# 0xMiden/miden-vm

Measured on NVIDIA H100. Metric: trace cells/sec proved, higher is better.
Workload: dtype u64

## Files before the change

miden-vm_b200/csrc/kernels.cu:

```cuda
#include "kernels.cuh"
#include "poseidon2.cuh"
#include "poseidon2_fast2.cuh"
#include "ntt2.cuh"
#include "blake3.cuh"
#include "keccak.cuh"
#include "rescue.cuh"
#include <algorithm>
#include <cstdio>

namespace mk {

static unsigned long long g_launches = 0;
unsigned long long launch_count() { return g_launches; }
void count_launch() { ++g_launches; }
void reset_launch_count() { g_launches = 0; }
#define COUNT_LAUNCH() (++g_launches)

void upload_constants() {
    cudaMemcpyToSymbol(p2::D_RC_EXT_INITIAL, p2::P2_RC_EXT_INITIAL, sizeof(u64) * 48);
    cudaMemcpyToSymbol(p2::D_RC_INTERNAL, p2::P2_RC_INTERNAL, sizeof(u64) * 22);
    cudaMemcpyToSymbol(p2::D_RC_EXT_TERMINAL, p2::P2_RC_EXT_TERMINAL, sizeof(u64) * 48);
    cudaMemcpyToSymbol(rsc::D_ARK1, rsc::RESCUE_ARK1, sizeof(u64) * 84);
    cudaMemcpyToSymbol(rsc::D_ARK2, rsc::RESCUE_ARK2, sizeof(u64) * 84);
}
// ... 51 lines not shown
        }
    }
}
void launch_push(const u64* src, const PeerPtrs& dst, u32 rank, u32 world, size_t n, cudaStream_t st) {
    if (!n || world <= 1) return;
    PushArgs a; a.src = src; a.dst = dst; a.rank = rank; a.world = world; a.n = n;
    unsigned blocks = (unsigned)std::min<size_t>((n / 2 + 255) / 256 + 1, 132 * 8);
    k_push<<<blocks, 256, 0, st>>>(a);
    COUNT_LAUNCH();
}

struct TransposeDst { PeerPtrs dst; PeerPtrs bad; u32 world; };
__global__ void k_transpose(const u64* __restrict__ src, TransposeDst d, u32 n_rows, u32 width, size_t col_stride, u32 row0) {
    __shared__ u64 tile[32][33];
    u32 r0 = blockIdx.x * 32, c0 = blockIdx.y * 32;
    bool any_bad = false;
    for (u32 i = threadIdx.y; i < 32; i += 8) {
        u32 r = r0 + i, c = c0 + threadIdx.x;
        if (r < n_rows && c < width) {
            u64 v = src[(size_t)r * width + c];
            any_bad |= (v >= gl::P);
            tile[i][threadIdx.x] = v;
        }
    }
    if (any_bad) for (u32 g = 0; g < d.world; g++) if (d.bad.p[g]) atomicOr(reinterpret_cast<u32*>(d.bad.p[g]), 1u);
    __syncthreads();
    for (u32 i = threadIdx.y; i < 32; i += 8) {
        u32 c = c0 + i, r = r0 + threadIdx.x;
        if (r < n_rows && c < width) {
            u64 v = tile[threadIdx.x][i];
            size_t o = (size_t)c * col_stride + row0 + r;
            for (u32 g = 0; g < d.world; g++) d.dst.p[g][o] = v;
        }
    }
}
void launch_transpose_rm_to_cm(const u64* src, u64* dst, u32 n_rows, u32 width, u32* d_bad_flag, cudaStream_t st) {
    TransposeDst d{}; d.dst.p[0] = dst; d.bad.p[0] = reinterpret_cast<u64*>(d_bad_flag); d.world = 1;
    dim3 grid((n_rows + 31) / 32, (width + 31) / 32), block(32, 8);
    k_transpose<<<grid, block, 0, st>>>(src, d, n_rows, width, (size_t)n_rows, 0u);
    COUNT_LAUNCH();
}
void launch_transpose_slice_push(const u64* src_slice, const PeerPtrs& dst_cm, const PeerPtrs& bad, u32 world, u32 row0, u32 n_rows_slice,
                                 u32 n_rows_total, u32 width, cudaStream_t st) {
    if (!n_rows_slice || !width) return;
    TransposeDst d{}; d.dst = dst_cm; d.bad = bad; d.world = world;
    dim3 grid((n_rows_slice + 31) / 32, (width + 31) / 32), block(32, 8);
    k_transpose<<<grid, block, 0, st>>>(src_slice, d, n_rows_slice, width, (size_t)n_rows_total, row0);
    COUNT_LAUNCH();
}

static constexpr int NTT_THREADS = 256;
static inline unsigned ntt_threads(u32 m, u32 log_cols) {
    u32 g = (m + log_cols >= 3) ? (1u << (m + log_cols - 3)) : 1u;
    if (g < 32) g = 32;
    if (g > 256) g = 256;
    return g;
}

__device__ __forceinline__ u64 w_pow(const u64* __restrict__ hi, const u64* __restrict__ lo, u32 lo_bits, u64 e) {
    return gl::mul(hi[e >> lo_bits], lo[e & ((1ull << lo_bits) - 1)]);
}

#define NTT_BOUNDS __launch_bounds__(NTT_THREADS)
template <int N1C, int N2C>
__global__ void NTT_BOUNDS k_intt_strided(u64* cols, size_t col_stride, NttTables T, u32 log_c) {
    extern __shared__ u64 sm[];
    ntt2::intt_strided_block<N1C, N2C>(blockIdx.x, blockIdx.y, sm, cols, col_stride, T, log_c);
}
template <int N2C>
__global__ void NTT_BOUNDS k_intt_contig(u64* cols, size_t col_stride, NttTables T) {
    extern __shared__ u64 sm[];
    ntt2::intt_contig_block<N2C>(blockIdx.x, blockIdx.y, sm, cols, col_stride, T);
}
template <int N1C, int N2C>
__global__ void NTT_BOUNDS k_fwd_contig(const FwdItem* __restrict__ items, NttTables T, PremulTables Pm) {
    extern __shared__ u64 sm[];
    ntt2::fwd_contig_block<N1C, N2C>(blockIdx.x, blockIdx.y, sm, items, T, Pm);
}
template <int N1C, int N2C>
__global__ void NTT_BOUNDS k_fwd_strided(const FwdItem* __restrict__ items, NttTables T, u32 log_c) {
    extern __shared__ u64 sm[];
    ntt2::fwd_strided_block<N1C, N2C>(blockIdx.x, blockIdx.y, sm, items, T, log_c);
}
#define NTT_SPECIALISED(X) X(8, 8) X(8, 9) X(9, 9) X(9, 10) X(10, 10) X(10, 11) X(11, 11)

template <int N1C, int N2C>
static void launch_intt_t(u64* cols, size_t col_stride, u32 n_cols, const NttTables& T, u32 log_c, cudaStream_t st) {
    u32 N1 = 1u << T.n1, N2 = 1u << T.n2, C = 1u << log_c;
    if (T.n1 > 0) {
        size_t smem = ntt2::smem_words_strided(T.n1, log_c) * sizeof(u64);
        cudaFuncSetAttribute(k_intt_strided<N1C, N2C>, cudaFuncAttributeMaxDynamicSharedMemorySize, (int)smem);
        k_intt_strided<N1C, N2C><<<dim3(N2 / C, n_cols), ntt_threads(T.n1, log_c), smem, st>>>(cols, col_stride, T, log_c);
        COUNT_LAUNCH();
    }
    size_t smem = ntt2::smem_words_contig_inv(T.n2) * sizeof(u64);
    k_intt_contig<N2C><<<dim3(N1, n_cols), ntt_threads(T.n2, 0), smem, st>>>(cols, col_stride, T);
    COUNT_LAUNCH();
}
void launch_intt(u64* cols, size_t col_stride, u32 n_cols, const NttTables& T, cudaStream_t st) {
    u32 log_c = T.n1 >= 12 ? 0 : 12 - T.n1; if (log_c > T.n2) log_c = T.n2;
#define X(a, b) if (T.n1 == a && T.n2 == b) { launch_intt_t<a, b>(cols, col_stride, n_cols, T, log_c, st); return; }
    NTT_SPECIALISED(X)
#undef X
    launch_intt_t<-1, -1>(cols, col_stride, n_cols, T, log_c, st);
}
template <int N1C, int N2C>
static void launch_fwd_t(const FwdItem* d_items, u32 n_items, const NttTables& T, const PremulTables& Pm, u32 log_c, cudaStream_t st) {
    u32 N1 = 1u << T.n1, N2 = 1u << T.n2, C = 1u << log_c;
    size_t smem = ntt2::smem_words_contig_fwd(T.n2) * sizeof(u64);
    k_fwd_contig<N1C, N2C><<<dim3(N1, n_items), ntt_threads(T.n2, 0), smem, st>>>(d_items, T, Pm);
    COUNT_LAUNCH();
    if (T.n1 > 0) {
        size_t smem2 = ntt2::smem_words_strided(T.n1, log_c) * sizeof(u64);
        cudaFuncSetAttribute(k_fwd_strided<N1C, N2C>, cudaFuncAttributeMaxDynamicSharedMemorySize, (int)smem2);
        k_fwd_strided<N1C, N2C><<<dim3(N2 / C, n_items), ntt_threads(T.n1, log_c), smem2, st>>>(d_items, T, log_c);
        COUNT_LAUNCH();
    }
}
void launch_fwd_ntt(const FwdItem* d_items, u32 n_items, const NttTables& T, const PremulTables& Pm, cudaStream_t st) {
    u32 log_c = T.n1 >= 12 ? 0 : 12 - T.n1; if (log_c > T.n2) log_c = T.n2;
#define X(a, b) if (T.n1 == a && T.n2 == b) { launch_fwd_t<a, b>(d_items, n_items, T, Pm, log_c, st); return; }
    NTT_SPECIALISED(X)
#undef X
    launch_fwd_t<-1, -1>(d_items, n_items, T, Pm, log_c, st);
}

static constexpr int HASH_THREADS = 128;
static constexpr int HASH_MIN_BLOCKS = 6;

enum { PERM_P2 = 0, PERM_RPO = 3, PERM_RPX = 4 };
template <int PERM>
__device__ __forceinline__ void alg_permute(u64* s) {
    if constexpr (PERM == PERM_RPO) rsc::rpo_permute(s);
    else if constexpr (PERM == PERM_RPX) rsc::rpx_permute(s);
    else p2f::permute(s);
}
#define ALG_BOUNDS(PERM) __launch_bounds__(HASH_THREADS, (PERM) == PERM_P2 ? HASH_MIN_BLOCKS : 1)
#define ALG_DISPATCH(perm, CALL) do { if ((perm) == PERM_RPO) { CALL(PERM_RPO); } else if ((perm) == PERM_RPX) { CALL(PERM_RPX); } else { CALL(PERM_P2); } } while (0)

template <int PERM>
__global__ void ALG_BOUNDS(PERM) k_leaf_hash(LeafArgs a, u32 log_n, u32 log_b, const u64* __restrict__ prev,
                                                            u32 prev_log_n, u64* __restrict__ states_out,
                                                            PushDst dig, u32 has_dig, u32 t0, u32 nt) {
    size_t L = (size_t)1 << (log_n + log_b);
    size_t idx = (size_t)blockIdx.x * blockDim.x + threadIdx.x;
    if (idx >= ((size_t)nt << log_n)) return;
    u32 t = t0 + (u32)(idx >> log_n);
    u32 r = (u32)(idx & (((size_t)1 << log_n) - 1));
    size_t pos = ((size_t)t << log_n) + r;
    u64 s[12];
    if (prev) {
        size_t Lp = (size_t)1 << (prev_log_n + log_b);
        size_t pp = ((size_t)t << prev_log_n) + (r & ((1u << prev_log_n) - 1));
#pragma unroll
        for (int k = 0; k < 12; k++) s[k] = prev[k * Lp + pp];
    } else {
#pragma unroll
        for (int k = 0; k < 12; k++) s[k] = 0;
    }
    for (int m = 0; m < a.n_mats; m++) {
        const u64* base = a.m[m].base + pos;
        u32 w = a.m[m].width;
        for (u32 c0 = 0; c0 < w; c0 += 8) {
#pragma unroll
            for (u32 k = 0; k < 8; k++) s[k] = (c0 + k < w) ? base[(size_t)(c0 + k) * L] : 0ull;
            alg_permute<PERM>(s);
        }
    }
    if (states_out) {
#pragma unroll
        for (int k = 0; k < 12; k++) states_out[k * L + pos] = glf::canon(s[k]);
    }
    if (has_dig) {
        size_t i = ((size_t)r << log_b) | t;
        push_u2(dig, 2 * i, i, make_ulonglong2(glf::canon(s[0]), glf::canon(s[1])));
        push_u2(dig, 2 * i + 1, i, make_ulonglong2(glf::canon(s[2]), glf::canon(s[3])));
    }
}
template <int PERM>
static void launch_leaf_hash_t(const LeafArgs& a, u32 log_n, u32 log_blowup, const u64* prev_states, u32 prev_log_n,
                               u64* states_out, const PushDst* dig, u32 t0, u32 nt, cudaStream_t st) {
    size_t cnt = (size_t)nt << log_n;
    unsigned blocks = (unsigned)((cnt + HASH_THREADS - 1) / HASH_THREADS);
    PushDst d = dig ? *dig : local_dst(nullptr);
    k_leaf_hash<PERM><<<blocks, HASH_THREADS, 0, st>>>(a, log_n, log_blowup, prev_states, prev_log_n, states_out, d, dig ? 1u : 0u, t0, nt);
    COUNT_LAUNCH();
}
void launch_leaf_hash(const LeafArgs& a, u32 log_n, u32 log_blowup, const u64* prev_states, u32 prev_log_n,
                      u64* states_out, const PushDst* dig, u32 t0, u32 nt, cudaStream_t st, int perm) {
#define X(PM) launch_leaf_hash_t<PM>(a, log_n, log_blowup, prev_states, prev_log_n, states_out, dig, t0, nt, st)
    ALG_DISPATCH(perm, X);
#undef X
}

template <int PERM>
__global__ void ALG_BOUNDS(PERM) k_compress(const u64* __restrict__ ch, u64* __restrict__ par, size_t n) {
    size_t i = (size_t)blockIdx.x * blockDim.x + threadIdx.x;
    if (i >= n) return;
    const ulonglong2* c = reinterpret_cast<const ulonglong2*>(ch + i * 8);
    ulonglong2 a0 = c[0], a1 = c[1], b0 = c[2], b1 = c[3];
    u64 s[12] = {a0.x, a0.y, a1.x, a1.y, b0.x, b0.y, b1.x, b1.y, 0, 0, 0, 0};
    alg_permute<PERM>(s);
    ulonglong2* d = reinterpret_cast<ulonglong2*>(par + i * 4);
    d[0] = make_ulonglong2(glf::canon(s[0]), glf::canon(s[1]));
    d[1] = make_ulonglong2(glf::canon(s[2]), glf::canon(s[3]));
}
template <int PERM>
// ... 856 lines not shown
```

miden-vm_b200/csrc/ntt_tables.hpp:

```cpp
#pragma once
#include "gl.cuh"
#include "kernels.cuh"
#include <vector>

namespace ntt_tables {
using gl::u64;
using gl::u32;

inline void split_n(u32 n, u32& n1, u32& n2) {
    if (n <= 11) { n1 = 0; n2 = n; }
    else { n1 = n / 2; n2 = n - n1; }
}
inline std::vector<u64> powers(u64 base, size_t count) {
    std::vector<u64> v(count);
    u64 x = 1;
    for (size_t i = 0; i < count; i++) { v[i] = x; x = gl::mul(x, base); }
    return v;
}

struct NttHost {
    u32 n, n1, n2, lo_bits;
    std::vector<u64> data;
    size_t o_tw1, o_twi1, o_twi2, o_lo, o_hi, o_ilo, o_ihi;
    mk::NttTables view(const u64* b) const {
        return mk::NttTables{n, n1, n2, lo_bits, b + o_tw1, b + o_twi1, b + o_twi2, b + o_lo, b + o_hi, b + o_ilo, b + o_ihi};
    }
};
inline NttHost build_ntt(u32 n) {
    NttHost h;
    h.n = n; split_n(n, h.n1, h.n2);
    h.lo_bits = (n + 1) / 2;
    u32 n1 = h.n1, n2 = h.n2, lo_bits = h.lo_bits;
    u64 w = gl::two_adic_generator(n), wi = gl::inv(w);
    auto push = [&](const std::vector<u64>& v) {
        if (h.data.size() & 1) h.data.push_back(0);
        size_t off = h.data.size(); h.data.insert(h.data.end(), v.begin(), v.end()); return off;
    };
    u64 w1 = gl::two_adic_generator(n1), w2 = gl::two_adic_generator(n2);
    h.o_tw1 = push(powers(w1, n1 ? (size_t)1 << (n1 - 1) : 1));
    h.o_twi1 = push(powers(gl::inv(w1), n1 ? (size_t)1 << (n1 - 1) : 1));
    h.o_twi2 = push(powers(gl::inv(w2), n2 ? (size_t)1 << (n2 - 1) : 1));
    h.o_lo = push(powers(w, (size_t)1 << lo_bits));
    h.o_hi = push(powers(gl::exp_pow2(w, lo_bits), (size_t)1 << (n - lo_bits)));
    h.o_ilo = push(powers(wi, (size_t)1 << lo_bits));
    h.o_ihi = push(powers(gl::exp_pow2(wi, lo_bits), (size_t)1 << (n - lo_bits)));
    return h;
}

struct PremulHost {
    u32 n_bases;
    std::vector<u64> data;
    size_t o_b, o_c;
    mk::PremulTables view(const u64* b) const { return mk::PremulTables{b + o_b, b + o_c}; }
};
inline PremulHost build_premul(const std::vector<u64>& bases, u32 n) {
    u32 n1, n2; split_n(n, n1, n2);
    size_t N1 = (size_t)1 << n1, N2 = (size_t)1 << n2, nb = bases.size();
    u64 n_inv = gl::inv((u64)1 << n);
    PremulHost h;
    h.n_bases = (u32)nb;
    h.o_b = 0; h.o_c = nb * N1;
    h.data.assign(nb * (N1 + N2), 0);
    for (size_t b = 0; b < nb; b++) {
        u64 g = bases[b], gN1 = gl::exp_pow2(g, n1);
        u64 x = n_inv;
        for (size_t j1 = 0; j1 < N1; j1++) { h.data[h.o_b + b * N1 + j1] = x; x = gl::mul(x, g); }
        u64* tc = &h.data[h.o_c + b * N2];
        for (u32 s = 0; s < n2; s++) {
            u64 shift = gl::exp_pow2(gN1, n2 - 1 - s), ws = gl::two_adic_generator(s + 1);
            u64 y = shift;
            for (size_t j = 0; j < ((size_t)1 << s); j++) { tc[(((size_t)1 << s) - 1) + j] = y; y = gl::mul(y, ws); }
        }
    }
    return h;
}

}
```

miden-vm_b200/csrc/session.cu:

```cuda
#include "../../include/miden_b200.h"
#include "host_transcript.hpp"
#include "kernels.cuh"
#include "ntt_tables.hpp"
#include "jit.hpp"
#include <cstddef>

#include <cstdarg>
#include <cstdio>
#include <cstring>
#include <functional>
#include <map>
#include <memory>
#include <stdexcept>
#include <string>
#include <thread>
#include <vector>

using gl::E2;
using gl::u32;
using gl::u64;
using hostfs::Duplex;
using hostfs::Indices;
using hostfs::Transcript;

// ... 180 lines not shown
        else mk::launch_compress_layer(children, parents, n, stream, perm());
    }
    mdn_external_check external_check = nullptr; void* external_ctx = nullptr;
    void shard_map_slab(char* base, size_t size);
    void shard_unmap_slabs();
    void shard_teardown();
    void shard_barrier();
    void shard_check(const char* where);
    u32 shard_flag_host = 0;
    void shard_check_enqueue();
    void shard_check_finish(const char* where);
    mk::PeerPtrs peers_of(const u64* p) const;
    mk::PushDst push_dst(u64* p, u32 mode, u32 owner_shift = 0) const;
    std::map<u32, std::unique_ptr<NttPlan>> ntt_plans;
    std::map<std::pair<u32, u32>, std::unique_ptr<PremulPlan>> premul_plans;

    Arena arena;
    bool use_arena = getenv("MDN_NO_ARENA") == nullptr;
    void release_proof_memory();
    bool in_proof = false;
    std::vector<AirHost> airs;
    std::vector<u32> log_heights;
    std::vector<u32> order;
    std::vector<u64> publics;
    u32 log_max_n = 0;
    u32 log_qd = 0;
    Transcript tr;
    std::vector<E2> randomness;
    Committed main_c, aux_c, quot_c;
    u32 jit_min_nodes = 256;
    std::map<u64, std::shared_ptr<jit::Kernel>> jit_kernels;
    std::vector<u64> jit_used;
    std::string jit_note;
    Committed prep_c; bool has_prep = false;
    std::vector<u32> prep_air, prep_log_h;
    void set_preprocessed(const mdn_statement* st, const mdn_matrix* mats);
    std::vector<std::vector<u64>> aux_values_p;
    DevBuf d_publics, d_randomness, d_aux_values, d_flag;
    void check_input_flag(const char* what);
    std::vector<size_t> aux_values_off;
    std::vector<uint8_t> out_heights;
    std::vector<u64> out_fields, out_commitments;
    E2 ood_z{0, 0};
    u64 dbg_roots[3][4] = {};
    std::vector<u64> dbg_quot_acc, dbg_deep, dbg_fri_roots, dbg_queries;
    bool keep_debug = false;
    mdn_timings timings{};
    cudaEvent_t ev[16];
    Prof prof;
    double leaf_bytes = 0, ntt_bytes = 0; unsigned long long perms = 0;

    NttPlan& ntt(u32 n);
    PremulPlan& premul_trace(u32 n);
    PremulPlan& premul_quotient(u32 n, u32 log_d);
    void build_tree(Committed& c);
    void lde_matrix(CommittedMat& m);
    void keep_raw_main(u32 j);
    void build_logup_aux(u32 j, u64* aux_cm, u64 final_out[2]);
    void lde_and_commit(Committed& c, float* t_lde, float* t_hash, bool lde_done = false);
    cudaStream_t copy_stream = nullptr;
    cudaEvent_t copy_ev[8];
    u64* bounce[2] = {nullptr, nullptr}; cudaEvent_t bounce_ev[2]; bool bounce_busy[2] = {false, false};
    static constexpr size_t BOUNCE_WORDS = (size_t)4 << 20;
    void host_to_device(u64* dst, const u64* src, size_t n);
    void upload_matrix(const mdn_matrix& m, bool on_device, u64* dst_cm);
    void prove_begin(const mdn_statement* st, const mdn_matrix* traces, const mdn_challenger* ch, u32 flags);
    void commit_aux(const mdn_matrix* aux, const u64* const* aux_values, bool zero_aux);
    void finish();
    u64 grind(u32 bits);
    void reset_proof();
};

namespace {

using ntt_tables::split_n;

}

NttPlan& mdn_session::ntt(u32 n) {
    auto it = ntt_plans.find(n);
    if (it != ntt_plans.end()) return *it->second;
    if (n > 22) fail(MDN_ERR_UNSUPPORTED, "trace height 2^%u exceeds the supported 2^22", n);
    auto plan = std::make_unique<NttPlan>();
    ntt_tables::NttHost host = ntt_tables::build_ntt(n);
    { ArenaScope persistent(nullptr); plan->store.alloc(host.data.size(), stream); }
    CUDA_OK(cudaMemcpyAsync(plan->store.p, host.data.data(), host.data.size() * sizeof(u64), cudaMemcpyHostToDevice, stream));
    CUDA_OK(cudaStreamSynchronize(stream));
    plan->T = host.view(plan->store.p);
    auto& ref = *plan;
    ntt_plans[n] = std::move(plan);
    return ref;
}

namespace {
std::unique_ptr<PremulPlan> make_premul(const std::vector<u64>& bases, u32 n, cudaStream_t stream) {
    ntt_tables::PremulHost host = ntt_tables::build_premul(bases, n);
    auto plan = std::make_unique<PremulPlan>();
    { ArenaScope persistent(nullptr); plan->store.alloc(host.data.size(), stream); }
    CUDA_OK(cudaMemcpyAsync(plan->store.p, host.data.data(), host.data.size() * sizeof(u64), cudaMemcpyHostToDevice, stream));
    CUDA_OK(cudaStreamSynchronize(stream));
    plan->P = host.view(plan->store.p);
    plan->n_bases = (u32)bases.size();
    return plan;
}
}

PremulPlan& mdn_session::premul_trace(u32 n) {
    auto key = std::make_pair(n, 0u);
    auto it = premul_plans.find(key);
    if (it != premul_plans.end()) return *it->second;
    u32 lb = params.log_blowup, B = 1u << lb;
    u64 s = gl::lde_shift(n + lb), wl = gl::two_adic_generator(n + lb);
    std::vector<u64> bases(B);
    u64 x = s;
    for (u32 t = 0; t < B; t++) { bases[t] = x; x = gl::mul(x, wl); }
    auto plan = make_premul(bases, n, stream);
    auto& ref = *plan;
    premul_plans[key] = std::move(plan);
    return ref;
}
PremulPlan& mdn_session::premul_quotient(u32 n, u32 log_d) {
    auto key = std::make_pair(n, 1u + log_d);
    auto it = premul_plans.find(key);
    if (it != premul_plans.end()) return *it->second;
    u32 lb = params.log_blowup, B = 1u << lb, D = 1u << log_d;
    u64 wl = gl::two_adic_generator(n + lb), wji = gl::inv(gl::two_adic_generator(n + log_d));
    std::vector<u64> bases(D * B);
    for (u32 t = 0; t < D; t++)
        for (u32 t2 = 0; t2 < B; t2++) bases[t * B + t2] = gl::mul(gl::pow(wji, t), gl::pow(wl, t2));
    auto plan = make_premul(bases, n, stream);
    auto& ref = *plan;
    premul_plans[key] = std::move(plan);
    return ref;
}

void mdn_session::reset_proof() {
    in_proof = false; shard_active = false;
    log_heights.clear(); order.clear(); publics.clear(); randomness.clear();
    aux_values_p.clear(); aux_values_off.clear();
    tr = Transcript();
    release_proof_memory();
}

void mdn_session::release_proof_memory() {
    main_c = Committed(); aux_c = Committed(); quot_c = Committed();
    airs.clear();
    d_publics.release(); d_randomness.release(); d_aux_values.release();
    arena.reset();
}

void mdn_session::shard_map_slab(char* base, size_t size) {
    if (shard_world <= 1) return;
    cudaIpcMemHandle_t h;
    CUDA_OK(cudaIpcGetMemHandle(&h, base));
    static_assert(sizeof(cudaIpcMemHandle_t) == 64, "CUDA IPC handle size");
    const size_t W = 10;
    std::vector<u64> mine(W), all(W * shard_world);
    memcpy(mine.data(), &h, 64); mine[8] = size; mine[9] = slab_views.size();
    if (allgather(allgather_ctx, mine.data(), all.data(), W) != 0) fail(MDN_ERR_INVALID_ARG, "all-gather callback failed");
    SlabView v{}; v.size = size;
    for (u32 g = 0; g < shard_world; g++) {
        if (all[g * W + 8] != size || all[g * W + 9] != mine[9])
            fail(MDN_ERR_INVALID_ARG, "rank %u allocated a different proof arena (slab %llu of %llu bytes here, slab %llu of %llu bytes there): every rank must prove the same statement with the same flags",
                 g, (unsigned long long)mine[9], (unsigned long long)size, (unsigned long long)all[g * W + 9], (unsigned long long)all[g * W + 8]);
        if (g == shard_rank) { v.base[g] = base; continue; }
        cudaIpcMemHandle_t hg; memcpy(&hg, &all[g * W], 64);
        void* m = nullptr;
        CUDA_OK(cudaIpcOpenMemHandle(&m, hg, cudaIpcMemLazyEnablePeerAccess));
        v.base[g] = (char*)m;
    }
    slab_views.push_back(v);
    { std::vector<u64> one(1, 0), got(shard_world); if (allgather(allgather_ctx, one.data(), got.data(), 1) != 0) fail(MDN_ERR_INVALID_ARG, "all-gather callback failed"); }
}
void mdn_session::shard_unmap_slabs() {
    if (slab_views.empty()) return;
    cudaStreamSynchronize(stream);
    for (auto& v : slab_views) for (u32 g = 0; g < shard_world; g++) if (g != shard_rank && v.base[g]) cudaIpcCloseMemHandle(v.base[g]);
    slab_views.clear();
    if (shard_world > 1 && allgather) { std::vector<u64> one(1, 0), all(shard_world); allgather(allgather_ctx, one.data(), all.data(), 1); }
// ... 47 lines not shown
    if (sharded()) CUDA_OK(cudaMemcpyAsync(&shard_flag_host, d_flag.p, sizeof shard_flag_host, cudaMemcpyDeviceToHost, stream));
}
void mdn_session::shard_check_finish(const char* where) {
    if (!sharded()) return;
    if (shard_flag_host & 8) { CUDA_OK(cudaMemsetAsync(d_flag.p, 0, 8, stream)); fail(MDN_ERR_CUDA, "cross-GPU barrier timed out (%s): a peer rank stopped or proves a different statement", where); }
}

void mdn_session::check_input_flag(const char* what) {
    u32 flag = 0;
    CUDA_OK(cudaMemcpyAsync(&flag, d_flag.p, sizeof flag, cudaMemcpyDeviceToHost, stream));
    CUDA_OK(cudaStreamSynchronize(stream));
    if (sharded()) {
        u32 peer_flag = 0;
        CUDA_OK(cudaMemcpyAsync(&peer_flag, sync_local + 16, sizeof peer_flag, cudaMemcpyDeviceToHost, stream));
        CUDA_OK(cudaStreamSynchronize(stream));
        if (peer_flag) { CUDA_OK(cudaMemsetAsync(sync_local + 16, 0, 8, stream)); flag |= peer_flag & 1u; }
    }
    if (flag) {
        CUDA_OK(cudaMemsetAsync(d_flag.p, 0, 8, stream));
        if (flag & 8) fail(MDN_ERR_CUDA, "cross-GPU barrier timed out: a peer rank stopped or proves a different statement");
        fail(MDN_ERR_INVALID_ARG, "%s contains a non-canonical field element (>= p)", what);
    }
}

void mdn_session::host_to_device(u64* dst, const u64* src, size_t n) {
    cudaPointerAttributes at{};
    bool pinned = cudaPointerGetAttributes(&at, src) == cudaSuccess && at.type == cudaMemoryTypeHost;
    cudaGetLastError();
    if (pinned) { CUDA_OK(cudaMemcpyAsync(dst, src, n * sizeof(u64), cudaMemcpyHostToDevice, copy_stream)); return; }
    for (int b = 0; b < 2; b++) if (!bounce[b]) { CUDA_OK(cudaHostAlloc((void**)&bounce[b], BOUNCE_WORDS * sizeof(u64), cudaHostAllocDefault)); CUDA_OK(cudaEventCreateWithFlags(&bounce_ev[b], cudaEventDisableTiming)); }
    unsigned nt = std::min(16u, std::max(1u, std::thread::hardware_concurrency() / 2));
    int b = 0;
    for (size_t off = 0; off < n; off += BOUNCE_WORDS, b ^= 1) {
        size_t cnt = std::min(BOUNCE_WORDS, n - off);
        if (bounce_busy[b]) CUDA_OK(cudaEventSynchronize(bounce_ev[b]));
        std::vector<std::thread> th;
        size_t per = (cnt + nt - 1) / nt;
        for (unsigned q = 0; q < nt; q++) {
            size_t a = (size_t)q * per, e = std::min(cnt, a + per);
            if (a >= e) break;
            th.emplace_back([=] { memcpy(bounce[b] + a, src + off + a, (e - a) * sizeof(u64)); });
        }
        for (auto& t : th) t.join();
        CUDA_OK(cudaMemcpyAsync(dst + off, bounce[b], cnt * sizeof(u64), cudaMemcpyHostToDevice, copy_stream));
        CUDA_OK(cudaEventRecord(bounce_ev[b], copy_stream));
        bounce_busy[b] = true;
    }
}

void mdn_session::upload_matrix(const mdn_matrix& m, bool on_device, u64* dst_cm) {
    size_t N = (size_t)1 << m.log_height;
    if (m.width == 0) return;
    if (on_device) {
        ProfScope ps(prof, PC_TRANSPOSE);
        mk::launch_transpose_rm_to_cm(m.values, dst_cm, (u32)N, m.width, (u32*)d_flag.p, stream);
        return;
    }
    DevBuf staging; staging.alloc(N * m.width, stream);
    CUDA_OK(cudaEventRecord(copy_ev[7], stream));
    CUDA_OK(cudaStreamWaitEvent(copy_stream, copy_ev[7], 0));
    host_to_device(staging.p, m.values, N * m.width);
    CUDA_OK(cudaEventRecord(copy_ev[6], copy_stream));
    CUDA_OK(cudaStreamWaitEvent(stream, copy_ev[6], 0));
    ProfScope ps(prof, PC_TRANSPOSE);
    mk::launch_transpose_rm_to_cm(staging.p, dst_cm, (u32)N, m.width, (u32*)d_flag.p, stream);
}

void mdn_session::lde_matrix(CommittedMat& m) {
    if (!m.width) return;
    u32 lb = params.log_blowup;
    size_t N = (size_t)1 << m.log_n, L = N << lb;
    NttPlan& plan = ntt(m.log_n);
    PremulPlan& pm = premul_trace(m.log_n);
    ProfScope ps(prof, PC_NTT);
    ntt_bytes += (double)(N + (size_t)nt() * N) * m.width * 8.0;
    if (sharded() && m.log_n >= shard_log_g + shard_min_log) {
        u32 c0 = (u32)((u64)m.width * shard_rank / shard_world), c1 = (u32)((u64)m.width * (shard_rank + 1) / shard_world);
        if (c1 > c0) mk::launch_intt(m.coef + (size_t)c0 * N, N, c1 - c0, plan.T, stream);
        shard_barrier();
        if (c1 > c0) mk::launch_push(m.coef + (size_t)c0 * N, peers_of(m.coef + (size_t)c0 * N), shard_rank, shard_world, (size_t)(c1 - c0) * N, stream);
        shard_barrier();
    } else mk::launch_intt(m.coef, N, m.width, plan.T, stream);
    const u32 tb = t0(), tn = nt();
    size_t col_bytes = (size_t)tn * N * sizeof(u64);
    u32 group = (u32)std::max<size_t>(1, (20u << 20) / col_bytes);
    std::vector<mk::FwdItem> items;
    for (u32 cc = 0; cc < m.width; cc++)
        for (u32 t = tb; t < tb + tn; t++)
            items.push_back(mk::FwdItem{m.coef + (size_t)cc * N, m.lde + (size_t)cc * L + (size_t)t * N, t, 0});
    DevBuf d_items;
    d_items.alloc(items.size() * sizeof(mk::FwdItem) / sizeof(u64), stream);
    CUDA_OK(cudaMemcpyAsync(d_items.p, items.data(), items.size() * sizeof(mk::FwdItem), cudaMemcpyHostToDevice, stream));
    for (u32 c0 = 0; c0 < m.width; c0 += group) {
        u32 cn = std::min(group, m.width - c0);
        mk::launch_fwd_ntt((const mk::FwdItem*)d_items.p + (size_t)c0 * tn, cn * tn, plan.T, pm.P, stream);
    }
}

void mdn_session::lde_and_commit(Committed& c, float* t_lde, float* t_hash, bool lde_done) {
    cudaEvent_t e0 = ev[12], e1 = ev[13], e2 = ev[14];
    CUDA_OK(cudaEventRecord(e0, stream));
    if (!lde_done) for (auto& m : c.mats) lde_matrix(m);
    CUDA_OK(cudaEventRecord(e1, stream));
    build_tree(c);
    CUDA_OK(cudaEventRecord(e2, stream));
    CUDA_OK(cudaEventSynchronize(e2));
    float a = 0, b = 0;
    cudaEventElapsedTime(&a, e0, e1); cudaEventElapsedTime(&b, e1, e2);
    if (t_lde) *t_lde += a;
    if (t_hash) *t_hash += b;
}

void mdn_session::build_tree(Committed& c) {
    u32 lb = params.log_blowup;
    u32 log_n_max = 0;
    for (auto& m : c.mats) log_n_max = std::max(log_n_max, m.log_n);
    u32 depth = log_n_max + lb;
    size_t L = (size_t)1 << depth;
    c.tree.depth = depth;
    c.tree.nodes.alloc((2 * L - 1) * 4, stream);
    const bool sh = sharded(), split = tree_sharded(depth);
    const u32 lg = shard_log_g, tb = t0(), tn = nt();
    mk::PushDst dig = push_dst(c.tree.layer(depth), sh ? (split ? mk::PUSH_OWNER : mk::PUSH_ALL) : mk::PUSH_LOCAL, depth - (split ? lg : 0));
    shard_barrier();
    DevBuf states_a, states_b;
    const u64* prev = nullptr; u32 prev_log = 0;
    size_t i = 0;
    while (i < c.mats.size()) {
        size_t j = i;
        mk::LeafArgs args; args.n_mats = 0;
        const u32 ln = c.mats[i].log_n;
        while (j < c.mats.size() && c.mats[j].log_n == ln && args.n_mats < 8) {
            if (c.mats[j].width || hash_kind == MDN_HASH_BLAKE3) args.m[args.n_mats++] = mk::LeafMat{c.mats[j].lde, c.mats[j].width, 0};
            j++;
        }
        bool last = (j == c.mats.size());
        DevBuf& out = (prev == states_a.p && prev) ? states_b : states_a;
        if (!last) out.alloc((size_t)state_words() << (ln + lb), stream);
        {
            ProfScope ps(prof, PC_LEAF);
            size_t Lg = (size_t)tn << ln;
            const u32 rate = hash_kind == MDN_HASH_KECCAK ? 17 : 8;
            for (int q = 0; q < args.n_mats; q++) { leaf_bytes += (double)Lg * args.m[q].width * 8.0; perms += Lg * ((args.m[q].width + rate - 1) / rate); }
            leaf_bytes += last ? (double)Lg * 32.0 : (double)Lg * 8.0 * state_words();
            hash_leaves(args, ln, lb, prev, prev_log, last ? nullptr : out.p, last ? &dig : nullptr, tb, tn);
        }
        prev = out.p; prev_log = ln;
        i = j;
    }
    shard_barrier();
    if (!split) {
        ProfScope ps(prof, PC_COMPRESS);
        perms += compress_subtree(c.tree, depth, 0, 0);
    } else {
        {
            ProfScope ps(prof, PC_COMPRESS);
            perms += compress_subtree(c.tree, depth, lg, shard_rank);
        }
        u64* mine = c.tree.layer(lg) + (size_t)shard_rank * 4;
        mk::launch_push(mine, peers_of(mine), shard_rank, shard_world, 4, stream);
        shard_barrier();
        ProfScope ps(prof, PC_COMPRESS);
        compress_subtree(c.tree, lg, 0, 0);
    }
    CUDA_OK(cudaMemcpyAsync(c.root, c.tree.layer(0), 4 * sizeof(u64), cudaMemcpyDeviceToHost, stream));
    shard_check_enqueue();
    CUDA_OK(cudaStreamSynchronize(stream));
    shard_check_finish("commitment");
}

u64 mdn_session::grind(u32 bits) {
    if (bits == 0) { tr.fields.push_back(0); return 0; }
    Duplex& ch = tr.ch;
    if (ch.hashed) {
        if (ch.bin.size() % (ch.keccak ? 8 : 4)) fail(MDN_ERR_INVALID_ARG, "hash challenger input buffer is not a whole number of words");
        u32 nw = (u32)(ch.bin.size() / 4);
        DevBuf d; d.alloc((nw + 1) / 2 + 2, stream);
        u64 none = ~0ull;
        if (nw) CUDA_OK(cudaMemcpyAsync(d.p + 1, ch.bin.data(), ch.bin.size(), cudaMemcpyHostToDevice, stream));
// ... 636 lines not shown
            try { air.jit->launch(ja, (unsigned)((own + 127) / 128), 128, stream); }
            catch (const std::exception& e) { fail(MDN_ERR_CUDA, "%s", e.what()); }
            mk::count_launch();
            if (air.jit->checked == 0) {
                DevBuf chk; chk.alloc(2 * Lj, stream);
                mk::ConstraintArgs cb = ca; cb.acc_out = chk.p;
                if (mk::launch_constraints(cb, stream) != 0) fail(MDN_ERR_UNSUPPORTED, "constraint program too large for the interpreter");
                for (u32 coord = 0; coord < 2; coord++) {
                    size_t o = (size_t)coord * Lj + ((size_t)ca.t0 << ln);
                    mk::launch_compare(chk.p + o, ca.acc_out + o, own, (u32*)d_flag.p, stream);
                }
                u32 flag = 0;
                CUDA_OK(cudaMemcpyAsync(&flag, d_flag.p, sizeof flag, cudaMemcpyDeviceToHost, stream));
                CUDA_OK(cudaStreamSynchronize(stream));
                if (sharded()) {
                    std::vector<u64> mine(1, flag & 4), all(shard_world);
                    if (allgather(allgather_ctx, mine.data(), all.data(), 1) != 0) fail(MDN_ERR_INVALID_ARG, "all-gather callback failed");
                    for (u64 f : all) flag |= (u32)f;
                }
                if (flag & 4) {
                    CUDA_OK(cudaMemsetAsync(d_flag.p, 0, 8, stream));
                    if (flag & ~4u) { u32 keep = flag & ~4u; CUDA_OK(cudaMemcpyAsync(d_flag.p, &keep, sizeof keep, cudaMemcpyHostToDevice, stream)); CUDA_OK(cudaStreamSynchronize(stream)); }
                    CUDA_OK(cudaMemcpyAsync(ca.acc_out, chk.p, 2 * Lj * sizeof(u64), cudaMemcpyDeviceToDevice, stream));
                    CUDA_OK(cudaStreamSynchronize(stream));
                    air.jit->checked = -1; jit_used.back() = 0;
                    jit_note = "NVRTC kernel disagreed with the interpreter on its first use; interpreter kept";
                } else air.jit->checked = 1;
            }
        } else if (mk::launch_constraints(ca, stream) != 0) fail(MDN_ERR_UNSUPPORTED, "constraint program too large for the interpreter");
        acc_cur = nxt; acc_prev_log = ln;
    }
    DevBuf acc = std::move(acc_pp[acc_cur]);
    acc_pp[1 - acc_cur].release();
    CUDA_OK(cudaEventRecord(ev[5], stream));
    const u32 tb = t0(), tn = nt();
    if (keep_debug) {
        if (sharded()) {
            shard_barrier();
            for (u32 coord = 0; coord < 2; coord++) { u64* own = acc.p + (size_t)coord * L + (size_t)tb * Nmax; mk::launch_push(own, peers_of(own), shard_rank, shard_world, (size_t)tn * Nmax, stream); }
            shard_barrier();
        }
        std::vector<u64> planes(2 * L);
        CUDA_OK(cudaMemcpyAsync(planes.data(), acc.p, 2 * L * sizeof(u64), cudaMemcpyDeviceToHost, stream));
        CUDA_OK(cudaStreamSynchronize(stream));
        u32 Dq = 1u << log_qd, cs = B >> log_qd;
        dbg_quot_acc.assign(2 * Nmax * Dq, 0);
        for (size_t t = 0; t < Dq; t++)
            for (size_t r = 0; r < Nmax; r++) {
                dbg_quot_acc[2 * (r * Dq + t)] = planes[t * cs * Nmax + r];
                dbg_quot_acc[2 * (r * Dq + t) + 1] = planes[L + t * cs * Nmax + r];
            }
    }
    const u32 D = 1u << log_qd, cstep = B >> log_qd;
    {
        NttPlan& plan = ntt(log_max_n);
        PremulPlan& pm = premul_quotient(log_max_n, log_qd);
        size_t rq = prof.begin(PC_NTT);
        ntt_bytes += (double)(Nmax + L) * 2 * D * 8.0 / (sharded() ? shard_world : 1);
        u32 c_lo = (tb + cstep - 1) / cstep, c_hi = std::min(D, (tb + tn + cstep - 1) / cstep);
        if (c_hi > c_lo)
            for (u32 coord = 0; coord < 2; coord++)
                mk::launch_intt(acc.p + (size_t)coord * L + (size_t)c_lo * cstep * Nmax, (size_t)cstep * Nmax, c_hi - c_lo, plan.T, stream);
        if (sharded()) {
            shard_barrier();
            for (u32 c = c_lo; c < c_hi; c++)
                for (u32 coord = 0; coord < 2; coord++) {
                    u64* chunk = acc.p + (size_t)coord * L + (size_t)c * cstep * Nmax;
                    mk::launch_push(chunk, peers_of(chunk), shard_rank, shard_world, Nmax, stream);
                }
            shard_barrier();
        }
        quot_c.lde_buf.alloc(L * 2 * D, stream);
        quot_c.coef_buf = std::move(acc);
        quot_c.mats.push_back(CommittedMat{quot_c.lde_buf.p, quot_c.coef_buf.p, log_max_n, 2 * D});
        std::vector<mk::FwdItem> items;
        for (u32 t = 0; t < D; t++)
            for (u32 coord = 0; coord < 2; coord++)
                for (u32 t2 = tb; t2 < tb + tn; t2++)
                    items.push_back(mk::FwdItem{quot_c.coef_buf.p + (size_t)coord * L + (size_t)t * cstep * Nmax,
                                                quot_c.lde_buf.p + (size_t)(2 * t + coord) * L + (size_t)t2 * Nmax, t * B + t2, 0});
        DevBuf d_items; d_items.alloc(items.size() * sizeof(mk::FwdItem) / sizeof(u64), stream);
        CUDA_OK(cudaMemcpyAsync(d_items.p, items.data(), items.size() * sizeof(mk::FwdItem), cudaMemcpyHostToDevice, stream));
        CUDA_OK(cudaStreamSynchronize(stream));
        u32 per = 2 * tn;
        u32 chunks_per_launch = std::max(1u, B / tn);
        for (u32 t = 0; t < D; t += chunks_per_launch) {
            u32 cn = std::min(chunks_per_launch, D - t);
            mk::launch_fwd_ntt((const mk::FwdItem*)d_items.p + (size_t)t * per, cn * per, plan.T, pm.P, stream);
        }
        prof.end(rq);
        build_tree(quot_c);
        tr.send_commitment(quot_c.root);
        memcpy(dbg_roots[2], quot_c.root, 32);
    }
    CUDA_OK(cudaEventRecord(ev[6], stream));
    u64 shift = gl::lde_shift(log_lde), shift_inv = gl::inv(shift);
    E2 z;
    for (;;) {
        z = tr.ch.sample_ext();
        if (z.a == 0 && z.b == 0) continue;
        if (gl::e2_eq(gl::e2_exp_pow2(z, log_max_n), gl::e2(1, 0))) continue;
        if (gl::e2_eq(gl::e2_exp_pow2(gl::e2_mulf(z, shift_inv), log_lde), gl::e2(1, 0))) continue;
        break;
    }
    ood_z = z;
    u64 omega_h = gl::two_adic_generator(log_max_n);
    E2 z_next = gl::e2_mulf(z, omega_h);

    std::vector<Committed*> groups;
    if (has_prep) groups.push_back(&prep_c);
    groups.push_back(&main_c); groups.push_back(&aux_c); groups.push_back(&quot_c);
    const int ng = (int)groups.size(), gq = ng - 1;
    struct MatEval { std::vector<u64> v; };
    std::vector<std::vector<MatEval>> evals(ng);
    {
        size_t ood_region = prof.begin(PC_OOD);
        size_t total_cols = 0;
        for (int g = 0; g < ng; g++) for (auto& cm : groups[g]->mats) total_cols += cm.width;
        const size_t T = std::max<size_t>(1, total_cols * 4);
        const u32 G = sharded() ? shard_world : 1, me = sharded() ? shard_rank : 0, lg = sharded() ? shard_log_g : 0;
        DevBuf d_all; d_all.alloc(T * G, stream);
        u64* d_out = d_all.p + (size_t)me * T;
        auto sliced = [&](u32 ln) { return G > 1 && ln >= lg + shard_min_log; };
        std::vector<DevBuf> keep;
        std::map<u32, std::pair<u64*, u64*>> weights;
        auto make_w = [&](u32 ln, E2 y0, E2 y1) {
            size_t S = sliced(ln) ? ((size_t)1 << (ln - lg)) : ((size_t)1 << ln), p0 = sliced(ln) ? S * me : 0;
            keep.emplace_back(); keep.back().alloc(2 * S, stream); u64* a = keep.back().p;
            keep.emplace_back(); keep.back().alloc(2 * S, stream); u64* b = keep.back().p;
            size_t tw = 2 * (((size_t)1 << (ln - ln / 2)) + ((size_t)1 << (ln / 2)));
            keep.emplace_back(); keep.back().alloc(2 * tw, stream); u64* sc = keep.back().p;
            mk::launch_pow_bitrev(y0, ln, a, sc, p0, S, stream);
            mk::launch_pow_bitrev(y1, ln, b, sc + tw, p0, S, stream);
            return std::make_pair(a, b);
        };
        size_t col_off = 0;
        struct Scale { size_t off; u64 n_inv; bool sliced; };
        std::vector<Scale> scale;
        for (int g = 0; g < ng; g++) {
            evals[g].resize(groups[g]->mats.size());
            for (size_t m = 0; m < groups[g]->mats.size(); m++) {
                CommittedMat& cm = groups[g]->mats[m];
                evals[g][m].v.assign((size_t)cm.width * 4, 0);
                if (!cm.width) continue;
                u32 ln = cm.log_n, lr = log_max_n - ln;
                size_t Nm = (size_t)1 << ln;
                const bool sl = sliced(ln);
                const u32 ls = sl ? ln - lg : ln;
                const size_t S = (size_t)1 << ls, s0 = sl ? S * me : 0;
                u32 n_chunks = (u32)std::max<size_t>(1, std::min<size_t>(S / 4096, 256));
                if (g != gq) {
                    auto it = weights.find(ln);
                    if (it == weights.end()) it = weights.emplace(ln, make_w(ln, gl::e2_exp_pow2(z, lr), gl::e2_exp_pow2(z_next, lr))).first;
                    keep.emplace_back(); keep.back().alloc((size_t)cm.width * n_chunks * 4, stream);
                    mk::launch_ood_dot(cm.coef + s0, Nm, cm.width, ls, it->second.first, it->second.second, keep.back().p, n_chunks, stream);
                    mk::launch_ood_reduce(keep.back().p, cm.width, n_chunks, d_out + col_off * 4, stream);
                } else {
                    u64 wj_inv = gl::inv(gl::two_adic_generator(log_max_n + log_qd));
                    for (u32 t = 0; t < D; t++) {
                        u64 f = gl::mul(shift_inv, gl::pow(wj_inv, t));
                        auto wv = make_w(ln, gl::e2_mulf(z, f), gl::e2_mulf(z_next, f));
                        keep.emplace_back(); keep.back().alloc((size_t)2 * n_chunks * 4, stream);
                        mk::launch_ood_dot(cm.coef + (size_t)t * cstep * Nm + s0, (size_t)B * Nm, 2, ls, wv.first, wv.second, keep.back().p, n_chunks, stream);
                        mk::launch_ood_reduce(keep.back().p, 2, n_chunks, d_out + (col_off + 2 * t) * 4, stream);
                    }
                }
                scale.push_back(Scale{col_off * 4, gl::inv((u64)Nm), sl});
                col_off += cm.width;
            }
        }
        prof.end(ood_region);
        if (G > 1) {
// ... 671 lines not shown
```

Measured before the change: 580.8 million.

## Cap strided NTT pass at 2^8 and slab forward NTT launches by bytes

Changes the four-step NTT split so that n1 is at most 8 (or n-12), which puts most of the size into a larger contiguous pass of up to 2^12 that lives in shared memory. The specialised template instances are updated to match. Forward-NTT batching moves into launch_fwd_ntt as byte-based slabs, so the callers' own grouping loops are dropped. Shared-memory opt-in is now only called above 48KB. The larger contiguous blocks need more shared memory per block, which may lower occupancy in exchange for a cheaper strided pass.

New measurement: 583.6 million (median of 6 runs). No clear change (+0.5%).

```diff
diff --git a/miden-vm_b200/csrc/kernels.cu b/miden-vm_b200/csrc/kernels.cu
--- a/miden-vm_b200/csrc/kernels.cu
+++ b/miden-vm_b200/csrc/kernels.cu
@@ -157,18 +157,24 @@
     extern __shared__ u64 sm[];
     ntt2::fwd_strided_block<N1C, N2C>(blockIdx.x, blockIdx.y, sm, items, T, log_c);
 }
-#define NTT_SPECIALISED(X) X(8, 8) X(8, 9) X(9, 9) X(9, 10) X(10, 10) X(10, 11) X(11, 11)
+#define NTT_SPECIALISED(X) X(8, 8) X(8, 9) X(8, 10) X(8, 11) X(8, 12) X(9, 12) X(10, 12)
+
+template <typename K>
+static void smem_opt_in(K kernel, size_t smem) {
+    if (smem > (48u << 10)) cudaFuncSetAttribute(kernel, cudaFuncAttributeMaxDynamicSharedMemorySize, (int)smem);
+}
 
 template <int N1C, int N2C>
 static void launch_intt_t(u64* cols, size_t col_stride, u32 n_cols, const NttTables& T, u32 log_c, cudaStream_t st) {
     u32 N1 = 1u << T.n1, N2 = 1u << T.n2, C = 1u << log_c;
     if (T.n1 > 0) {
         size_t smem = ntt2::smem_words_strided(T.n1, log_c) * sizeof(u64);
-        cudaFuncSetAttribute(k_intt_strided<N1C, N2C>, cudaFuncAttributeMaxDynamicSharedMemorySize, (int)smem);
+        smem_opt_in(k_intt_strided<N1C, N2C>, smem);
         k_intt_strided<N1C, N2C><<<dim3(N2 / C, n_cols), ntt_threads(T.n1, log_c), smem, st>>>(cols, col_stride, T, log_c);
         COUNT_LAUNCH();
     }
     size_t smem = ntt2::smem_words_contig_inv(T.n2) * sizeof(u64);
+    smem_opt_in(k_intt_contig<N2C>, smem);
     k_intt_contig<N2C><<<dim3(N1, n_cols), ntt_threads(T.n2, 0), smem, st>>>(cols, col_stride, T);
     COUNT_LAUNCH();
 }
@@ -183,21 +189,27 @@
 static void launch_fwd_t(const FwdItem* d_items, u32 n_items, const NttTables& T, const PremulTables& Pm, u32 log_c, cudaStream_t st) {
     u32 N1 = 1u << T.n1, N2 = 1u << T.n2, C = 1u << log_c;
     size_t smem = ntt2::smem_words_contig_fwd(T.n2) * sizeof(u64);
+    smem_opt_in(k_fwd_contig<N1C, N2C>, smem);
     k_fwd_contig<N1C, N2C><<<dim3(N1, n_items), ntt_threads(T.n2, 0), smem, st>>>(d_items, T, Pm);
     COUNT_LAUNCH();
     if (T.n1 > 0) {
         size_t smem2 = ntt2::smem_words_strided(T.n1, log_c) * sizeof(u64);
-        cudaFuncSetAttribute(k_fwd_strided<N1C, N2C>, cudaFuncAttributeMaxDynamicSharedMemorySize, (int)smem2);
+        smem_opt_in(k_fwd_strided<N1C, N2C>, smem2);
         k_fwd_strided<N1C, N2C><<<dim3(N2 / C, n_items), ntt_threads(T.n1, log_c), smem2, st>>>(d_items, T, log_c);
         COUNT_LAUNCH();
     }
 }
+static constexpr size_t FWD_SLAB_BYTES = (size_t)24 << 20;
 void launch_fwd_ntt(const FwdItem* d_items, u32 n_items, const NttTables& T, const PremulTables& Pm, cudaStream_t st) {
     u32 log_c = T.n1 >= 12 ? 0 : 12 - T.n1; if (log_c > T.n2) log_c = T.n2;
-#define X(a, b) if (T.n1 == a && T.n2 == b) { launch_fwd_t<a, b>(d_items, n_items, T, Pm, log_c, st); return; }
-    NTT_SPECIALISED(X)
+    size_t slab = std::max<size_t>(1, FWD_SLAB_BYTES >> (T.n + 3));
+    for (u32 i = 0; i < n_items; i += (u32)slab) {
+        u32 cnt = (u32)std::min<size_t>(slab, n_items - i);
+#define X(a, b) if (T.n1 == a && T.n2 == b) { launch_fwd_t<a, b>(d_items + i, cnt, T, Pm, log_c, st); continue; }
+        NTT_SPECIALISED(X)
 #undef X
-    launch_fwd_t<-1, -1>(d_items, n_items, T, Pm, log_c, st);
+        launch_fwd_t<-1, -1>(d_items + i, cnt, T, Pm, log_c, st);
+    }
 }
 
 static constexpr int HASH_THREADS = 128;
diff --git a/miden-vm_b200/csrc/ntt_tables.hpp b/miden-vm_b200/csrc/ntt_tables.hpp
--- a/miden-vm_b200/csrc/ntt_tables.hpp
+++ b/miden-vm_b200/csrc/ntt_tables.hpp
@@ -10,6 +10,10 @@
 inline void split_n(u32 n, u32& n1, u32& n2) {
     if (n <= 11) { n1 = 0; n2 = n; }
     else { n1 = n / 2; n2 = n - n1; }
+}
+inline u32 plan_n1(u32 n) {
+    u32 n1, n2; split_n(n, n1, n2);
+    return n1 <= 8 ? n1 : (n - 12 > 8 ? n - 12 : 8);
 }
 inline std::vector<u64> powers(u64 base, size_t count) {
     std::vector<u64> v(count);
@@ -26,9 +30,9 @@
         return mk::NttTables{n, n1, n2, lo_bits, b + o_tw1, b + o_twi1, b + o_twi2, b + o_lo, b + o_hi, b + o_ilo, b + o_ihi};
     }
 };
-inline NttHost build_ntt(u32 n) {
+inline NttHost build_ntt(u32 n, u32 n1_split) {
     NttHost h;
-    h.n = n; split_n(n, h.n1, h.n2);
+    h.n = n; h.n1 = n1_split; h.n2 = n - n1_split;
     h.lo_bits = (n + 1) / 2;
     u32 n1 = h.n1, n2 = h.n2, lo_bits = h.lo_bits;
     u64 w = gl::two_adic_generator(n), wi = gl::inv(w);
@@ -46,6 +50,7 @@
     h.o_ihi = push(powers(gl::exp_pow2(wi, lo_bits), (size_t)1 << (n - lo_bits)));
     return h;
 }
+inline NttHost build_ntt(u32 n) { u32 n1, n2; split_n(n, n1, n2); return build_ntt(n, n1); }
 
 struct PremulHost {
     u32 n_bases;
@@ -53,8 +58,8 @@
     size_t o_b, o_c;
     mk::PremulTables view(const u64* b) const { return mk::PremulTables{b + o_b, b + o_c}; }
 };
-inline PremulHost build_premul(const std::vector<u64>& bases, u32 n) {
-    u32 n1, n2; split_n(n, n1, n2);
+inline PremulHost build_premul(const std::vector<u64>& bases, u32 n, u32 n1) {
+    u32 n2 = n - n1;
     size_t N1 = (size_t)1 << n1, N2 = (size_t)1 << n2, nb = bases.size();
     u64 n_inv = gl::inv((u64)1 << n);
     PremulHost h;
@@ -74,5 +79,6 @@
     }
     return h;
 }
+inline PremulHost build_premul(const std::vector<u64>& bases, u32 n) { u32 n1, n2; split_n(n, n1, n2); return build_premul(bases, n, n1); }
 
 }
diff --git a/miden-vm_b200/csrc/session.cu b/miden-vm_b200/csrc/session.cu
--- a/miden-vm_b200/csrc/session.cu
+++ b/miden-vm_b200/csrc/session.cu
@@ -286,7 +286,7 @@
     if (it != ntt_plans.end()) return *it->second;
     if (n > 22) fail(MDN_ERR_UNSUPPORTED, "trace height 2^%u exceeds the supported 2^22", n);
     auto plan = std::make_unique<NttPlan>();
-    ntt_tables::NttHost host = ntt_tables::build_ntt(n);
+    ntt_tables::NttHost host = ntt_tables::build_ntt(n, ntt_tables::plan_n1(n));
     { ArenaScope persistent(nullptr); plan->store.alloc(host.data.size(), stream); }
     CUDA_OK(cudaMemcpyAsync(plan->store.p, host.data.data(), host.data.size() * sizeof(u64), cudaMemcpyHostToDevice, stream));
     CUDA_OK(cudaStreamSynchronize(stream));
@@ -298,7 +298,7 @@
 
 namespace {
 std::unique_ptr<PremulPlan> make_premul(const std::vector<u64>& bases, u32 n, cudaStream_t stream) {
-    ntt_tables::PremulHost host = ntt_tables::build_premul(bases, n);
+    ntt_tables::PremulHost host = ntt_tables::build_premul(bases, n, ntt_tables::plan_n1(n));
     auto plan = std::make_unique<PremulPlan>();
     { ArenaScope persistent(nullptr); plan->store.alloc(host.data.size(), stream); }
     CUDA_OK(cudaMemcpyAsync(plan->store.p, host.data.data(), host.data.size() * sizeof(u64), cudaMemcpyHostToDevice, stream));
@@ -512,8 +512,6 @@
         shard_barrier();
     } else mk::launch_intt(m.coef, N, m.width, plan.T, stream);
     const u32 tb = t0(), tn = nt();
-    size_t col_bytes = (size_t)tn * N * sizeof(u64);
-    u32 group = (u32)std::max<size_t>(1, (20u << 20) / col_bytes);
     std::vector<mk::FwdItem> items;
     for (u32 cc = 0; cc < m.width; cc++)
         for (u32 t = tb; t < tb + tn; t++)
@@ -521,10 +519,7 @@
     DevBuf d_items;
     d_items.alloc(items.size() * sizeof(mk::FwdItem) / sizeof(u64), stream);
     CUDA_OK(cudaMemcpyAsync(d_items.p, items.data(), items.size() * sizeof(mk::FwdItem), cudaMemcpyHostToDevice, stream));
-    for (u32 c0 = 0; c0 < m.width; c0 += group) {
-        u32 cn = std::min(group, m.width - c0);
-        mk::launch_fwd_ntt((const mk::FwdItem*)d_items.p + (size_t)c0 * tn, cn * tn, plan.T, pm.P, stream);
-    }
+    mk::launch_fwd_ntt((const mk::FwdItem*)d_items.p, (u32)items.size(), plan.T, pm.P, stream);
 }
 
 void mdn_session::lde_and_commit(Committed& c, float* t_lde, float* t_hash, bool lde_done) {
@@ -1327,12 +1322,7 @@
         DevBuf d_items; d_items.alloc(items.size() * sizeof(mk::FwdItem) / sizeof(u64), stream);
         CUDA_OK(cudaMemcpyAsync(d_items.p, items.data(), items.size() * sizeof(mk::FwdItem), cudaMemcpyHostToDevice, stream));
         CUDA_OK(cudaStreamSynchronize(stream));
-        u32 per = 2 * tn;
-        u32 chunks_per_launch = std::max(1u, B / tn);
-        for (u32 t = 0; t < D; t += chunks_per_launch) {
-            u32 cn = std::min(chunks_per_launch, D - t);
-            mk::launch_fwd_ntt((const mk::FwdItem*)d_items.p + (size_t)t * per, cn * per, plan.T, pm.P, stream);
-        }
+        mk::launch_fwd_ntt((const mk::FwdItem*)d_items.p, (u32)items.size(), plan.T, pm.P, stream);
         prof.end(rq);
         build_tree(quot_c);
         tr.send_commitment(quot_c.root);
```
